# numericalEFT/FeynmanDiagram.jl

Hardware: AMD Instinct MI355X
Metric: graph-evaluations/sec (higher is better)
Workload: dtype f64

## Files before the change

### feynmandiagram.jl_amd/csrc/fdg_binned.hip

```cpp
#include <hip/hip_runtime.h>

#include <algorithm>
#include <cmath>
#include <mutex>
#include <type_traits>
#include <utility>
#include <vector>

#define FDG_RUNTIME_TU 1
#include "fdg_internal.h"
#include "fdg_matsubara.h"
#include "fdg_sincos.h"

using namespace fdg;

namespace {

constexpr uint32_t kBinWaves = 4;
constexpr size_t kBinLdsBudget = 64u << 10;
constexpr size_t kBinSlabBytes = 64ull << 20;
constexpr uint32_t kKeyInvalid = 0xFFFFFFC0u;

__device__ inline void bin_barrier() {
  __asm__ volatile("s_waitcnt lgkmcnt(0)\n\ts_barrier" ::: "memory");
}

__device__ inline uint32_t wave_sort_keys(uint32_t &key, uint32_t lane, uint64_t valid) {
  const uint32_t key0 = __shfl(key, 0);
  if (valid == ~0ull && __ballot((key >> 6) == (key0 >> 6)) == ~0ull) return lane;
#pragma unroll
  for (uint32_t kb = 2; kb <= 64; kb <<= 1)
#pragma unroll
    for (uint32_t jb = kb >> 1; jb > 0; jb >>= 1) {
      const uint32_t other = __shfl_xor(key, (int)jb);
      const bool keep_min = ((lane & kb) == 0) == ((lane & jb) == 0);
      key = keep_min ? min(key, other) : max(key, other);
    }
  return key & 63u;
}

__device__ inline void wave_runs(uint32_t key, uint32_t lane, uint32_t &j, bool &head, uint32_t &end) {
  j = key >> 6;
  const bool ok = key < kKeyInvalid;
  const uint32_t j_prev = __shfl_up(j, 1);
  const uint32_t j_next = __shfl_down(j, 1);
  head = ok && (lane == 0 || j_prev != j);
  const uint64_t tails = __ballot(!ok || lane == 63 || j_next != j);
  end = ok ? (uint32_t)__builtin_ctzll(tails & (~0ull << lane)) : lane;
}

struct SegTiles { long t0, t1, rounds; };
__device__ inline SegTiles seg_tiles_of(long n, uint32_t seg, long seg_tiles) {
  const long ntile = (n + 63) / 64, t0 = (long)seg * seg_tiles, t1 = min(t0 + seg_tiles, ntile);
  return {t0, t1, t1 > t0 ? (t1 - t0 + kBinWaves - 1) / kBinWaves : 0};
}

enum BinMode { kFirst = 0, kBoth = 1, kSplit = 2 };

constexpr uint32_t kGrpCols = FDG_WEIGHT_GROUP_MAX, kGrpEntry = 1u + kGrpCols + 16u;

template <int RS, int MODE, bool GRP = false>
__global__ void __launch_bounds__(256)
fdg_binned_partials(const double *__restrict__ root, long ld, long n, const int32_t *__restrict__ bins, int32_t bin_base, uint32_t n_bin,
                    const double *__restrict__ weight, uint32_t R, uint32_t n_slice, long seg_tiles, double *__restrict__ partial, int first,
                    const uint32_t *__restrict__ gtab, long wstride) {
  extern __shared__ double hist[];
  constexpr uint32_t NH = MODE == kBoth ? 2 : 1;
  const uint32_t lane = threadIdx.x & 63u, wave = threadIdx.x >> 6;
  const uint32_t n_grp = MODE == kSplit ? 2 * n_slice : n_slice;
  const uint32_t grp = blockIdx.x % n_grp, seg = blockIdx.x / n_grp;
  const uint32_t mom = MODE == kSplit ? grp / n_slice : 0, slice = grp % n_slice;
  const uint32_t k0 = slice * RS, kn = min((uint32_t)RS, R - k0);
  const size_t hist_cols = (size_t)n_bin * R;
  double *slab = partial + (size_t)seg * hist_cols * (MODE == kFirst ? 1 : 2) + (size_t)mom * hist_cols + k0;
  for (uint32_t i = threadIdx.x; i < NH * n_bin * RS; i += 256) {
    const uint32_t j = i / RS, kk = i % RS;
    hist[i] = (first || kk >= kn) ? 0.0 : slab[(size_t)j * R + kk];
  }
  __syncthreads();
  const SegTiles sg = seg_tiles_of(n, seg, seg_tiles);
  const long t0 = sg.t0, t1 = sg.t1, rounds = sg.rounds;

  constexpr int WC = !GRP ? 1 : RS < (int)kGrpCols ? RS : (int)kGrpCols;
  uint32_t n_wcol = 1, wcol[WC] = {}, widx[RS] = {};
  if constexpr (GRP) {
    const uint32_t *e = gtab + R + (size_t)slice * kGrpEntry;
    n_wcol = e[0];
#pragma unroll
    for (int c = 0; c < WC; ++c) wcol[c] = e[1 + c];
#pragma unroll
    for (int kk = 0; kk < RS; ++kk) widx[kk] = e[1 + kGrpCols + kk];
  }
  int32_t bin_n;
  double w_n[WC] = {}, r_n[RS];
  auto fetch = [&](long r) {
    const long b = min((t0 + r * (long)kBinWaves + wave) * 64 + lane, n - 1);
    bin_n = bins ? bins[b] : bin_base;
    if constexpr (GRP) {
#pragma unroll
      for (int c = 0; c < WC; ++c)
        if ((uint32_t)c < n_wcol) w_n[c] = weight[(size_t)wcol[c] * (size_t)wstride + (size_t)b];
    } else {
      w_n[0] = weight ? weight[b] : 1.0;
    }
#pragma unroll
    for (int kk = 0; kk < RS; ++kk) r_n[kk] = root[(size_t)min(k0 + kk, R - 1) * (size_t)ld + (size_t)b];
  };
  fetch(0);
  for (long r = 0; r < rounds; ++r) {
    const long t = t0 + r * (long)kBinWaves + wave, b = t * 64 + lane;
    const int64_t jb = (int64_t)bin_n - (int64_t)bin_base;
    const bool in = t < t1 && b < n && jb >= 0 && jb < (int64_t)n_bin;
    uint32_t key = in ? ((uint32_t)jb << 6) | lane : kKeyInvalid | lane;
    double v[RS];
#pragma unroll
    for (int kk = 0; kk < RS; ++kk) {
      double wk = w_n[0];
#pragma unroll
      for (int c = 1; c < WC; ++c) wk = widx[kk] == (uint32_t)c ? w_n[c] : wk;
      v[kk] = in ? wk * r_n[kk] : 0.0;
    }
    fetch(r + 1);

    const uint64_t valid = __ballot(key < kKeyInvalid);
    double s[RS] = {}, s2[RS] = {};
    bool head = false;
    uint32_t j = 0;
    if (valid) {
      const uint32_t src = wave_sort_keys(key, lane, valid);
      uint32_t end;
      wave_runs(key, lane, j, head, end);
#pragma unroll
      for (int kk = 0; kk < RS; ++kk) s[kk] = __shfl(v[kk], (int)src);
      if (MODE == kBoth) {
#pragma unroll
        for (int kk = 0; kk < RS; ++kk) s2[kk] = s[kk] * s[kk];
      } else if (MODE == kSplit && mom) {
#pragma unroll
        for (int kk = 0; kk < RS; ++kk) s[kk] = s[kk] * s[kk];
      }
      for (uint32_t d = 1; d < 64; d <<= 1) {
        const bool take = lane + d <= end;
        if (!__ballot(take)) break;
#pragma unroll
        for (int kk = 0; kk < RS; ++kk) {
          const double t = __shfl_down(s[kk], d);
          if (take) s[kk] = s[kk] + t;
        }
        if (MODE == kBoth) {
#pragma unroll
          for (int kk = 0; kk < RS; ++kk) {
            const double t = __shfl_down(s2[kk], d);
            if (take) s2[kk] = s2[kk] + t;
          }
        }
      }
    }
    for (uint32_t w = 0; w < kBinWaves; ++w) {
      if (wave == w && head) {
#pragma unroll
        for (int kk = 0; kk < RS; ++kk)
          if ((uint32_t)kk < kn) {
            hist[j * RS + kk] = hist[j * RS + kk] + s[kk];
            if (MODE == kBoth) hist[(n_bin + j) * RS + kk] = hist[(n_bin + j) * RS + kk] + s2[kk];
          }
      }
      bin_barrier();
    }
  }
  __syncthreads();
  for (uint32_t i = threadIdx.x; i < NH * n_bin * RS; i += 256) {
    const uint32_t jj = i / RS, kk = i % RS;
    if (kk < kn) slab[(size_t)jj * R + kk] = hist[i];
  }
}

__global__ void __launch_bounds__(256)
fdg_binned_reduce(const double *__restrict__ partial, uint32_t n_seg, long seg_stride, long ncol, uint32_t R, uint32_t C,
                  double *__restrict__ acc, double *__restrict__ acc2, const uint8_t *__restrict__ live) {
  __shared__ double sh[256];
  const uint32_t Q = 256u / C, q = threadIdx.x / C, cl = threadIdx.x % C;
  const long c = (long)blockIdx.x * C + cl;
  const double *part = partial + (size_t)blockIdx.y * (size_t)ncol;
  double *out = blockIdx.y ? acc2 : acc;
  double s = 0.0;
  if (c < ncol)
    for (uint32_t sg = q; sg < n_seg; sg += Q) s = s + part[(size_t)sg * (size_t)seg_stride + (size_t)c];
  sh[threadIdx.x] = s;
  __syncthreads();
  if (q == 0 && c < ncol) {
    double t = sh[cl];
    for (uint32_t qq = 1; qq < Q && qq < n_seg; ++qq) t = t + sh[qq * C + cl];
    if (!live || live[c % R]) out[c] = out[c] + t;
  }
}

constexpr uint32_t kObsGroup = 16;
constexpr uint32_t kObsNone = 0xFFFFFFFFu;
constexpr uint32_t kObsFirst = 0x80000000u;

__global__ void __launch_bounds__(256)
fdg_obs_partials(const double *__restrict__ root, long ld, long n, const int32_t *__restrict__ bins, int32_t bin_base, uint32_t n_bin,
                 const double *__restrict__ weight, long wstride, uint32_t n_wcol, uint32_t V, uint32_t CS, uint32_t n_slice, long seg_tiles,
                 double *__restrict__ partial, int first, const uint32_t *__restrict__ utab, const double *__restrict__ dtab) {
  extern __shared__ double hist[];
  const uint32_t lane = threadIdx.x & 63u, wave = threadIdx.x >> 6;
  const uint32_t slice = blockIdx.x % n_slice, seg = blockIdx.x / n_slice;
  const uint32_t c0 = slice * CS, cn = min(CS, V - c0);
  const uint32_t *hdr = utab + (size_t)slice * 4u;
  const uint32_t n_rec = hdr[1];
  const uint32_t *colA = utab + hdr[2], *colB = colA + CS, *rec = colB + CS, *tslot = rec + (size_t)n_rec * 4u;
  const double *tcoef = dtab + hdr[3];
  double *stash = hist + (size_t)n_bin * CS + threadIdx.x;
  double *slab = partial + (size_t)seg * n_bin * V + c0;
  for (uint32_t i = threadIdx.x; i < n_bin * CS; i += 256) {
    const uint32_t j = i / CS, cl = i % CS;
    hist[i] = (first || cl >= cn) ? 0.0 : slab[(size_t)j * V + cl];
  }
  __syncthreads();
  const SegTiles sg = seg_tiles_of(n, seg, seg_tiles);
  const long t0 = sg.t0, t1 = sg.t1, rounds = sg.rounds;
  int32_t bin_n;
  auto fetch = [&](long r) {
    const long b = min((t0 + r * (long)kBinWaves + wave) * 64 + lane, n - 1);
    bin_n = bins ? bins[b] : bin_base;
  };
  fetch(0);
  for (long r = 0; r < rounds; ++r) {
    const long t = t0 + r * (long)kBinWaves + wave, b = t * 64 + lane;
    const int64_t jb = (int64_t)bin_n - (int64_t)bin_base;
    const bool in = t < t1 && b < n && jb >= 0 && jb < (int64_t)n_bin;
    uint32_t key = in ? ((uint32_t)jb << 6) | lane : kKeyInvalid | lane;
    fetch(r + 1);
    const uint64_t valid = __ballot(key < kKeyInvalid);
    bool head = false, ok = false;
    uint32_t j = 0, end = lane;
    if (valid) {
      const uint32_t src = wave_sort_keys(key, lane, valid);
      wave_runs(key, lane, j, head, end);
      ok = key < kKeyInvalid;
      const size_t bs = (size_t)min(t * 64 + (long)src, n - 1);
      double wv[kGrpCols] = {};
#pragma unroll
      for (uint32_t c = 0; c < kGrpCols; ++c)
        if (c < n_wcol) wv[c] = weight[(size_t)c * (size_t)wstride + bs];
      for (uint32_t i0 = 0; i0 < n_rec; i0 += 4) {
        double rv[4];
#pragma unroll
        for (uint32_t u = 0; u < 4; ++u) rv[u] = root[(size_t)rec[(size_t)min(i0 + u, n_rec - 1u) * 4u] * (size_t)ld + bs];
#pragma unroll
        for (uint32_t u = 0; u < 4; ++u) {
          if (i0 + u >= n_rec) break;
          const uint32_t *e = rec + (size_t)(i0 + u) * 4u;
          const uint32_t wc = e[1];
          double wk = wv[0];
#pragma unroll
          for (uint32_t c = 1; c < kGrpCols; ++c) wk = wc == c ? wv[c] : wk;
          const double tk = n_wcol ? wk * rv[u] : rv[u];
          for (uint32_t ti = e[2]; ti < e[3]; ++ti) {
            const uint32_t sl = tslot[ti];
            double *o = stash + (size_t)(sl & ~kObsFirst) * 256u;
            const double p = tcoef[ti] * tk;
            *o = (sl & kObsFirst) ? p : *o + p;
          }
        }
      }
    }
    for (uint32_t g0 = 0; g0 < cn; g0 += kObsGroup) {
      double s[kObsGroup];
      if (valid) {
#pragma unroll
        for (uint32_t i = 0; i < kObsGroup; ++i) {
          const uint32_t cl = min(g0 + i, cn - 1u), a = colA[cl], c = colB[cl];
          double v = 0.0;
          if (a != kObsNone) {
            v = stash[(size_t)a * 256u];
            if (c != kObsNone) v = v * stash[(size_t)c * 256u];
          }
          s[i] = ok ? v : 0.0;
        }
        for (uint32_t d = 1; d < 64; d <<= 1) {
          const bool take = lane + d <= end;
          if (!__ballot(take)) break;
#pragma unroll
          for (uint32_t i = 0; i < kObsGroup; ++i) {
            const double up = __shfl_down(s[i], d);
            if (take) s[i] = s[i] + up;
          }
        }
      }
      for (uint32_t w = 0; w < kBinWaves; ++w) {
        if (wave == w && head) {
#pragma unroll
          for (uint32_t i = 0; i < kObsGroup; ++i)
            if (g0 + i < cn) hist[(size_t)j * CS + g0 + i] = hist[(size_t)j * CS + g0 + i] + s[i];
        }
        bin_barrier();
      }
    }
  }
  __syncthreads();
  for (uint32_t i = threadIdx.x; i < n_bin * CS; i += 256) {
    const uint32_t jj = i / CS, cl = i % CS;
    if (cl < cn) slab[(size_t)jj * V + cl] = hist[i];
  }
}

__global__ void __launch_bounds__(256)
fdg_obs_reduce(const double *__restrict__ partial, uint32_t n_seg, long ncol, uint32_t n_obs, uint32_t V, uint32_t C, uint32_t rowlive,
               double *__restrict__ obs, double *__restrict__ cov) {
  __shared__ double sh[256];
  const uint32_t Q = 256u / C, q = threadIdx.x / C, cl = threadIdx.x % C;
  const long c = (long)blockIdx.x * C + cl;
  double s = 0.0;
  if (c < ncol)
    for (uint32_t sg = q; sg < n_seg; sg += Q) s = s + partial[(size_t)sg * (size_t)ncol + (size_t)c];
  sh[threadIdx.x] = s;
  __syncthreads();
  if (q == 0 && c < ncol) {
    double t = sh[cl];
    for (uint32_t qq = 1; qq < Q && qq < n_seg; ++qq) t = t + sh[qq * C + cl];
    const size_t jb = (size_t)(c / V);
    const uint32_t v = (uint32_t)(c % V);
    if (v < n_obs) {
      if ((rowlive >> v) & 1u) obs[jb * n_obs + v] = obs[jb * n_obs + v] + t;
    } else {
      uint32_t a = 0, p = v - n_obs;
      while (p >= n_obs - a) { p -= n_obs - a; ++a; }
      const uint32_t cc = a + p;
      if (((rowlive >> a) & 1u) && ((rowlive >> cc) & 1u)) {
        double *m = cov + jb * n_obs * n_obs;
        const double up = m[a * n_obs + cc] + t;
        m[a * n_obs + cc] = up;
        if (cc != a) m[cc * n_obs + a] = m[cc * n_obs + a] + t;
      }
    }
  }
}

constexpr uint32_t kFobsRec = 6;
constexpr uint32_t kFobsSame = 0x80000000u;
constexpr uint32_t kFobsIm = 0x40000000u;

__global__ void __launch_bounds__(256)
fdg_fobs_partials(const double *__restrict__ root, long ld, long n, const int32_t *__restrict__ bins, int32_t bin_base, uint32_t n_bin,
                  const double *__restrict__ weight, long wstride, uint32_t n_wcol, const double *__restrict__ T, long ts, long tc,
                  double beta, uint32_t n_freq, uint32_t FS, uint32_t n_fslice, uint32_t V, uint32_t CS, uint32_t n_cslice, long seg_tiles,
                  double *__restrict__ partial, int first, const uint32_t *__restrict__ utab, const double *__restrict__ dtab) {
  extern __shared__ double hist[];
  const uint32_t lane = threadIdx.x & 63u, wave = threadIdx.x >> 6;
  const uint32_t n_grp = n_fslice * n_cslice, grp = blockIdx.x % n_grp, seg = blockIdx.x / n_grp;
// ... 126 lines not shown
                double *__restrict__ fobs, double *__restrict__ fcov) {
  __shared__ double sh[256];
  const uint32_t Q = 256u / C, q = threadIdx.x / C, cl = threadIdx.x % C;
  const long c = (long)blockIdx.x * C + cl;
  double s = 0.0;
  if (c < ncol)
    for (uint32_t sg = q; sg < n_seg; sg += Q) s = s + partial[(size_t)sg * (size_t)ncol + (size_t)c];
  sh[threadIdx.x] = s;
  __syncthreads();
  if (q == 0 && c < ncol) {
    double t = sh[cl];
    for (uint32_t qq = 1; qq < Q && qq < n_seg; ++qq) t = t + sh[qq * C + cl];
    const size_t row = (size_t)(c / V);
    const uint32_t v = (uint32_t)(c % V);
    if (v < n_comp) {
      if ((live >> v) & 1u) fobs[row * n_comp + v] = fobs[row * n_comp + v] + t;
    } else {
      uint32_t a = 0, p = v - n_comp;
      while (p >= n_comp - a) { p -= n_comp - a; ++a; }
      const uint32_t cc = a + p;
      if (((live >> a) & 1u) && ((live >> cc) & 1u)) {
        double *m = fcov + row * n_comp * n_comp;
        m[a * n_comp + cc] = m[a * n_comp + cc] + t;
        if (cc != a) m[cc * n_comp + a] = m[cc * n_comp + a] + t;
      }
    }
  }
}

__device__ __forceinline__ uint32_t vegas_cell(uint64_t sample, uint32_t d, uint64_t seed, uint32_t G, double &y) {
  const double u = fdg_philox_u53(sample, d, seed);
  y = u * (double)G;
  return min((uint32_t)(int)y, G - 1u);
}

struct VegasStrat { uint32_t n[FDG_VEGAS_DIM_MAX], div[FDG_VEGAS_DIM_MAX], H; };

__device__ __forceinline__ uint32_t vegas_cell_strat(uint64_t sample, uint32_t d, uint64_t seed, uint32_t G, uint32_t s, uint32_t ns, double &y) {
  const double u = fdg_philox_u53(sample, d, seed);
  const double v = ((double)s + u) / (double)ns;
  y = v * (double)G;
  return min((uint32_t)(int)y, G - 1u);
}

struct VegasCols { uint32_t c[FDG_VEGAS_DIM_MAX]; };

struct VegasNoFold { __device__ void operator()(uint32_t, double) const {} };
struct VegasPlainCell {
  __device__ __forceinline__ uint32_t operator()(uint64_t sample, uint32_t d, uint64_t seed, uint32_t G, double &y) const {
    return vegas_cell(sample, d, seed, G, y);
  }
};
struct VegasStratCell {
  const VegasStrat *sv;
  uint32_t rem;
  __device__ __forceinline__ uint32_t operator()(uint64_t sample, uint32_t d, uint64_t seed, uint32_t G, double &y) {
    const uint32_t ns = sv->n[d], sd = rem % ns;
    rem /= ns;
    return vegas_cell_strat(sample, d, seed, G, sd, ns, y);
  }
};
template <bool kPolar = false, class Fold = VegasNoFold, class Cell = VegasPlainCell>
__device__ __forceinline__ double vegas_draw(const double *__restrict__ grid, uint32_t D, uint32_t G, const VegasCols &col, uint64_t seed,
                                             uint64_t off, double *__restrict__ x, long xs, long xc, int32_t *__restrict__ cell, long n, long b,
                                             uint64_t grouped = 0, double *stash = nullptr, Fold fold = Fold(), Cell pick = Cell()) {
  double jb = 0.0;
  uint32_t slot = 0;
  for (uint32_t d = 0; d < D; ++d) {
    double y;
    const uint32_t c = pick(off + (uint64_t)b, d, seed, G, y);
    const double *e = grid + (size_t)d * (G + 1u) + c;
    const double lo = e[0], wd = e[1] - lo, fr = y - (double)c;
    const double v = lo + fr * wd;
    if (kPolar && ((grouped >> d) & 1u)) stash[(slot++) * 256u + threadIdx.x] = v;
    else x[b * xs + (long)col.c[d] * xc] = v;
    const double f = (double)G * wd;
    jb = d ? jb * f : f;
    fold(d, f);
    if (cell) cell[(size_t)d * (size_t)n + (size_t)b] = (int32_t)c;
  }
  return jb;
}

__global__ void __launch_bounds__(256)
fdg_vegas_sample(const double *__restrict__ grid, uint32_t D, uint32_t G, VegasCols col, uint64_t seed, uint64_t off, double *__restrict__ x,
                 long xs, long xc, double *__restrict__ jac, int32_t *__restrict__ cell, long n) {
  for (long b = blockIdx.x * 256L + threadIdx.x; b < n; b += (long)gridDim.x * 256L) {
    const double jb = vegas_draw(grid, D, G, col, seed, off, x, xs, xc, cell, n, b);
    jac[b] = jb;
  }
}

__global__ void __launch_bounds__(256)
fdg_vegas_sample_strat(const double *__restrict__ grid, uint32_t D, uint32_t G, VegasCols col, VegasStrat sv, const int64_t *__restrict__ start,
                       uint64_t seed, uint64_t off, double *__restrict__ x, long xs, long xc, double *__restrict__ jac,
                       int32_t *__restrict__ cube, int32_t *__restrict__ cell, long n) {
  const uint32_t H = sv.H;
  const int64_t n_total = start[H];
  for (long b = blockIdx.x * 256L + threadIdx.x; b < n; b += (long)gridDim.x * 256L) {
    const int64_t i = (int64_t)(off + (uint64_t)b);
    uint32_t lo = 0, hi = H - 1u;
    while (lo < hi) {
      const uint32_t mid = (lo + hi + 1u) >> 1;
      if (start[mid] <= i) lo = mid; else hi = mid - 1u;
    }
    const int64_t n_h = start[lo + 1u] - start[lo];
    cube[b] = (int32_t)lo;
    uint32_t rem = lo;
    double jb = 0.0;
    for (uint32_t d = 0; d < D; ++d) {
      const uint32_t ns = sv.n[d], sd = rem % ns;
      rem /= ns;
      double y;
      const uint32_t c = vegas_cell_strat(off + (uint64_t)b, d, seed, G, sd, ns, y);
      const double *e = grid + (size_t)d * (G + 1u) + c;
      const double el = e[0], wd = e[1] - el, fr = y - (double)c;
      x[b * xs + (long)col.c[d] * xc] = el + fr * wd;
      const double f = (double)G * wd;
      jb = d ? jb * f : f;
      if (cell) cell[(size_t)d * (size_t)n + (size_t)b] = (int32_t)c;
    }
    const double fac = (double)n_total / ((double)H * (double)n_h);
    jac[b] = jb * fac;
  }
}

struct VegasExtCols { uint32_t c[FDG_VEGAS_EXT_MAX]; };

__device__ __forceinline__ double vegas_pick_discrete(const double *__restrict__ cdf, uint32_t n_bin, int32_t bin_base,
                                                      const double *__restrict__ ext, uint32_t n_ext, const VegasExtCols &ecol, uint64_t seed,
                                                      uint64_t off, uint32_t D, double *__restrict__ x, long xs, long xc,
                                                      int32_t *__restrict__ bin, long b) {
  const double u = fdg_philox_u53(off + (uint64_t)b, D, seed);
  uint32_t lo = 0, hi = n_bin - 1u;
  while (lo < hi) {
    const uint32_t mid = (lo + hi) >> 1;
    if (cdf[mid + 1u] <= u) lo = mid + 1u; else hi = mid;
  }
  const double p = cdf[lo + 1u] - cdf[lo];
  bin[b] = (int32_t)lo + bin_base;
  for (uint32_t e = 0; e < n_ext; ++e) x[b * xs + (long)ecol.c[e] * xc] = ext[(size_t)lo * n_ext + e];
  return p;
}

__device__ __forceinline__ void vegas_draw_discrete(const double *__restrict__ cdf, uint32_t n_bin, int32_t bin_base,
                                                    const double *__restrict__ ext, uint32_t n_ext, const VegasExtCols &ecol, uint64_t seed,
                                                    uint64_t off, uint32_t D, double *__restrict__ x, long xs, long xc,
                                                    double *__restrict__ jac, int32_t *__restrict__ bin, long b, double jb) {
  const double p = vegas_pick_discrete(cdf, n_bin, bin_base, ext, n_ext, ecol, seed, off, D, x, xs, xc, bin, b);
  jac[b] = jb / p;
}

__global__ void __launch_bounds__(256)
fdg_vegas_sample_discrete(const double *__restrict__ grid, uint32_t D, uint32_t G, VegasCols col, const double *__restrict__ cdf,
                          uint32_t n_bin, int32_t bin_base, const double *__restrict__ ext, uint32_t n_ext, VegasExtCols ecol, uint64_t seed,
                          uint64_t off, double *__restrict__ x, long xs, long xc, double *__restrict__ jac, int32_t *__restrict__ bin,
                          int32_t *__restrict__ cell, long n) {
  for (long b = blockIdx.x * 256L + threadIdx.x; b < n; b += (long)gridDim.x * 256L) {
    const double jb = vegas_draw(grid, D, G, col, seed, off, x, xs, xc, cell, n, b);
    vegas_draw_discrete(cdf, n_bin, bin_base, ext, n_ext, ecol, seed, off, D, x, xs, xc, jac, bin, b, jb);
  }
}

struct VegasPolar {
  uint64_t grouped;
  uint32_t n;
  uint32_t var[FDG_VEGAS_POLAR_MAX], dim[FDG_VEGAS_POLAR_MAX];
  uint32_t col[FDG_VEGAS_POLAR_MAX][3];
};

struct VegasGroupMasks {
  uint64_t m[FDG_WEIGHT_GROUP_MAX];
  uint32_t n;
};

struct VegasNoStrat {};
struct VegasStratArgs {
  VegasStrat sv;
  const int64_t *start;
  int32_t *cube;
};
template <bool GRP, bool STRAT = false>
__global__ void __launch_bounds__(256)
fdg_vegas_sample_polar(const double *__restrict__ grid, uint32_t D, uint32_t G, VegasCols col, VegasPolar pol, const double *__restrict__ cdf,
                       uint32_t n_bin, int32_t bin_base, const double *__restrict__ ext, uint32_t n_ext, VegasExtCols ecol, uint64_t seed,
                       uint64_t off, double *__restrict__ x, long xs, long xc, double *__restrict__ jac, int32_t *__restrict__ bin,
                       int32_t *__restrict__ cell, long n, VegasGroupMasks gm, long jstride,
                       std::conditional_t<STRAT, VegasStratArgs, VegasNoStrat> sa) {
  extern __shared__ double polar_stash[];
  constexpr int NG = GRP ? FDG_WEIGHT_GROUP_MAX : 1;
  for (long b = blockIdx.x * 256L + threadIdx.x; b < n; b += (long)gridDim.x * 256L) {
    [[maybe_unused]] double fac = 1.0;
    [[maybe_unused]] uint32_t hcube = 0;
    if constexpr (STRAT) {
      const uint32_t H = sa.sv.H;
      const int64_t i = (int64_t)(off + (uint64_t)b);
      uint32_t lo = 0, hi = H - 1u;
      while (lo < hi) {
        const uint32_t mid = (lo + hi + 1u) >> 1;
        if (sa.start[mid] <= i) lo = mid; else hi = mid - 1u;
      }
      const int64_t n_h = sa.start[lo + 1u] - sa.start[lo];
      sa.cube[b] = (int32_t)lo;
      hcube = lo;
      fac = (double)sa.start[H] / ((double)H * (double)n_h);
    }
    double jg[NG];
#pragma unroll
    for (int g = 0; g < NG; ++g) jg[g] = 1.0;
    auto fold = [&](uint32_t d, double f) {
      if constexpr (GRP) {
#pragma unroll
        for (int g = 0; g < NG; ++g)
          if ((uint32_t)g < gm.n && ((gm.m[g] >> d) & 1u)) jg[g] = jg[g] * f;
      }
    };
    double jb;
    if constexpr (STRAT) jb = vegas_draw<true>(grid, D, G, col, seed, off, x, xs, xc, cell, n, b, pol.grouped, polar_stash, fold, VegasStratCell{&sa.sv, hcube});
    else jb = vegas_draw<true>(grid, D, G, col, seed, off, x, xs, xc, cell, n, b, pol.grouped, polar_stash, fold);
    for (uint32_t g = 0; g < pol.n; ++g) {
      const uint32_t var = pol.var[g];
      const double *v = polar_stash + (size_t)__popcll(pol.grouped & ((1ull << var) - 1ull)) * 256u + threadIdx.x;
      double *xb = x + b * xs;
      const double k = v[0];
      double sp, cp, st = 0.0;
      if (pol.dim[g] == 3) {
        double ct;
        fdg_sincos_impl(v[256], st, ct);
        fdg_sincos_impl(v[512], sp, cp);
        const double ks = k * st;
        xb[(long)pol.col[g][0] * xc] = ks * cp;
        xb[(long)pol.col[g][1] * xc] = ks * sp;
        xb[(long)pol.col[g][2] * xc] = k * ct;
        jb = jb * k;
        jb = jb * k;
        jb = jb * st;
      } else {
        fdg_sincos_impl(v[256], sp, cp);
        xb[(long)pol.col[g][0] * xc] = k * cp;
        xb[(long)pol.col[g][1] * xc] = k * sp;
        jb = jb * k;
      }
      if constexpr (GRP) {
#pragma unroll
        for (int h = 0; h < NG; ++h)
          if ((uint32_t)h < gm.n && ((gm.m[h] >> var) & 1u)) {
            jg[h] = jg[h] * k;
            if (pol.dim[g] == 3) {
              jg[h] = jg[h] * k;
              jg[h] = jg[h] * st;
            }
          }
      }
    }
    if constexpr (STRAT) {
      if constexpr (GRP) {
#pragma unroll
        for (int g = 0; g < NG; ++g)
          if ((uint32_t)g < gm.n) jac[(size_t)g * (size_t)jstride + (size_t)b] = jg[g] * fac;
      } else {
        jac[b] = jb * fac;
      }
    } else if constexpr (GRP) {
      const double p = cdf ? vegas_pick_discrete(cdf, n_bin, bin_base, ext, n_ext, ecol, seed, off, D, x, xs, xc, bin, b) : 1.0;
#pragma unroll
      for (int g = 0; g < NG; ++g)
        if ((uint32_t)g < gm.n) jac[(size_t)g * (size_t)jstride + (size_t)b] = cdf ? jg[g] / p : jg[g];
    } else {
      if (!cdf) { jac[b] = jb; continue; }
      vegas_draw_discrete(cdf, n_bin, bin_base, ext, n_ext, ecol, seed, off, D, x, xs, xc, jac, bin, b, jb);
    }
  }
}

__device__ __forceinline__ double vegas_term(const double *__restrict__ root, long ld, size_t bb, const double *__restrict__ weight,
                                             const uint32_t *__restrict__ kidx, const double *__restrict__ coef, uint32_t n_live) {
  double sum = 0.0;
  for (uint32_t i = 0; i < n_live; ++i) {
    const double rk = root[(size_t)kidx[i] * (size_t)ld + bb];
    const double term = coef ? coef[i] * rk : rk;
    sum = i ? sum + term : term;
  }
  return weight ? weight[bb] * sum : sum;
}

__device__ __forceinline__ double vegas_group_term(const double *__restrict__ root, long ld, size_t bb, const double *__restrict__ weight,
                                                   long wstride, const uint32_t *__restrict__ kidx, const double *__restrict__ coef,
                                                   const uint32_t *__restrict__ gstart, uint32_t g) {
  const uint32_t i0 = gstart[g], i1 = gstart[g + 1u];
  return vegas_term(root, ld, bb, weight + (size_t)g * (size_t)wstride, kidx + i0, coef ? coef + i0 : nullptr, i1 - i0);
}

struct VegasVarGroups { uint8_t g[FDG_VEGAS_DIM_MAX]; };

template <int BINNED, bool GRP = false, bool STRAT = false>
__global__ void __launch_bounds__(256)
fdg_vegas_partials(const double *__restrict__ root, long ld, long n, const double *__restrict__ weight, const uint32_t *__restrict__ kidx,
                   const double *__restrict__ coef, uint32_t n_live, uint64_t seed, uint64_t off, uint32_t D, uint32_t G, uint32_t DS,
                   uint32_t n_slice, long seg_tiles, double *__restrict__ partial, int first, const int32_t *__restrict__ bins,
                   int32_t bin_base, uint32_t n_bin, const uint32_t *__restrict__ gstart, uint32_t NG, long wstride, VegasVarGroups vgm,
                   const int32_t *__restrict__ cube, VegasStrat sv) {
  extern __shared__ double hist[];
  const uint32_t vtile = GRP ? NG * 64u : 64u;
  const uint32_t lane = threadIdx.x & 63u, wave = threadIdx.x >> 6;
  const uint32_t slice = blockIdx.x % n_slice, seg = blockIdx.x / n_slice;
  const uint32_t d0 = slice * DS, dn = min(DS, D - d0);
  double *vbuf = hist + (size_t)DS * G;
  double *slab = partial + ((size_t)seg * D + d0) * G;
  for (uint32_t i = threadIdx.x; i < dn * G; i += 256) hist[i] = first ? 0.0 : slab[i];
  __syncthreads();
  const SegTiles sg = seg_tiles_of(n, seg, seg_tiles);
  const long t0 = sg.t0, t1 = sg.t1, rounds = sg.rounds;
  for (long r = 0; r < rounds; ++r) {
    {
      const long t = t0 + r * (long)kBinWaves + wave, b = t * 64 + lane;
      bool in = t < t1 && b < n;
      const size_t bb = (size_t)min(b, n - 1);
      if (BINNED) {
        const int64_t jb = (int64_t)bins[bb] - (int64_t)bin_base;
        in = in && jb >= 0 && jb < (int64_t)n_bin;
      }
      const double out = (BINNED && t < t1 && b < n) ? -1.0 : 0.0;
      double *vb = vbuf + ((r & 1) * kBinWaves + wave) * vtile + lane;
      if constexpr (GRP) {
        for (uint32_t g = 0; g < NG; ++g) {
          const double tw = vegas_group_term(root, ld, bb, weight, wstride, kidx, coef, gstart, g);
          vb[g * 64u] = in ? tw * tw : out;
        }
      } else {
        const double tw = vegas_term(root, ld, bb, weight, kidx, coef, n_live);
        vb[0] = in ? tw * tw : out;
      }
    }
    __syncthreads();
    for (uint32_t tt = 0; tt < kBinWaves; ++tt) {
      const long t = t0 + r * (long)kBinWaves + tt, b = t * 64 + lane;
      if (t >= t1) break;
      const double *vb = vbuf + ((r & 1) * kBinWaves + tt) * vtile + lane;
      double v = GRP ? 0.0 : vb[0];
      uint32_t hc = 0;
      if constexpr (STRAT) hc = (uint32_t)cube[(size_t)min(b, n - 1)];
      for (uint32_t dd = wave; dd < dn; dd += kBinWaves) {
        if constexpr (GRP) {
          const uint32_t owners = vgm.g[d0 + dd];
          if (!owners) continue;
          bool any = false;
          for (uint32_t g = 0; g < NG; ++g)
            if ((owners >> g) & 1u) {
              const double q = vb[g * 64u];
              v = any ? v + q : q;
              any = true;
            }
        }
        double y;
        uint32_t c;
        if constexpr (STRAT) c = vegas_cell_strat(off + (uint64_t)b, d0 + dd, seed, G, hc / sv.div[d0 + dd] % sv.n[d0 + dd], sv.n[d0 + dd], y);
        else c = vegas_cell(off + (uint64_t)b, d0 + dd, seed, G, y);
        uint32_t key = (b < n && !(STRAT && hc >= sv.H) && !(BINNED && v < 0.0)) ? (c << 6) | lane : kKeyInvalid | lane;
        const uint64_t valid = __ballot(key < kKeyInvalid);
        if (!valid) continue;
        const uint32_t src = wave_sort_keys(key, lane, valid);
        uint32_t j, end;
        bool head;
        wave_runs(key, lane, j, head, end);
        double s = __shfl(v, (int)src);
        for (uint32_t dist = 1; dist < 64; dist <<= 1) {
          const bool take = lane + dist <= end;
          if (!__ballot(take)) break;
          const double up = __shfl_down(s, dist);
          if (take) s = s + up;
        }
        if (head) hist[dd * G + j] = hist[dd * G + j] + s;
      }
    }
  }
  __syncthreads();
  for (uint32_t i = threadIdx.x; i < dn * G; i += 256) slab[i] = hist[i];
}

template <bool GRP = false>
__global__ void __launch_bounds__(256)
fdg_vegas_bin_partials(const double *__restrict__ root, long ld, long n, const int32_t *__restrict__ bins, int32_t bin_base, uint32_t n_bin,
                       const double *__restrict__ weight, const uint32_t *__restrict__ kidx, const double *__restrict__ coef, uint32_t n_live,
                       long seg_tiles, double *__restrict__ partial, int first, const uint32_t *__restrict__ gstart, uint32_t NG,
                       long wstride) {
  extern __shared__ double hist[];
  const uint32_t lane = threadIdx.x & 63u, wave = threadIdx.x >> 6;
  const uint32_t seg = blockIdx.x;
  double *slab = partial + (size_t)seg * n_bin;
  for (uint32_t i = threadIdx.x; i < n_bin; i += 256) hist[i] = first ? 0.0 : slab[i];
  __syncthreads();
  const SegTiles sg = seg_tiles_of(n, seg, seg_tiles);
  const long t0 = sg.t0, t1 = sg.t1, rounds = sg.rounds;
  int32_t bin_n;
  double t_n = 0.0;
  auto fetch = [&](long r) {
    const size_t bb = (size_t)min((t0 + r * (long)kBinWaves + wave) * 64 + lane, n - 1);
    bin_n = bins[bb];
    if constexpr (GRP) {
      bool any = false;
      for (uint32_t g = 0; g < NG; ++g) {
        if (gstart[g] == gstart[g + 1u]) continue;
        const double tw = vegas_group_term(root, ld, bb, weight, wstride, kidx, coef, gstart, g), q = tw * tw;
        t_n = any ? t_n + q : q;
        any = true;
      }
    } else {
      t_n = vegas_term(root, ld, bb, weight, kidx, coef, n_live);
    }
  };
  fetch(0);
  for (long r = 0; r < rounds; ++r) {
    const long t = t0 + r * (long)kBinWaves + wave, b = t * 64 + lane;
    const int64_t jb = (int64_t)bin_n - (int64_t)bin_base;
    const bool in = t < t1 && b < n && jb >= 0 && jb < (int64_t)n_bin;
    uint32_t key = in ? ((uint32_t)jb << 6) | lane : kKeyInvalid | lane;
    const double v = in ? (GRP ? t_n : t_n * t_n) : 0.0;
    fetch(r + 1);
    const uint64_t valid = __ballot(key < kKeyInvalid);
    double s = 0.0;
    bool head = false;
    uint32_t j = 0;
    if (valid) {
      const uint32_t src = wave_sort_keys(key, lane, valid);
      uint32_t end;
      wave_runs(key, lane, j, head, end);
      s = __shfl(v, (int)src);
      for (uint32_t dist = 1; dist < 64; dist <<= 1) {
        const bool take = lane + dist <= end;
        if (!__ballot(take)) break;
        const double up = __shfl_down(s, dist);
        if (take) s = s + up;
      }
    }
    for (uint32_t w = 0; w < kBinWaves; ++w) {
      if (wave == w && head) hist[j] = hist[j] + s;
      bin_barrier();
    }
  }
  __syncthreads();
  for (uint32_t i = threadIdx.x; i < n_bin; i += 256) slab[i] = hist[i];
}

template <int KW, bool HSPLIT, bool GRP = false>
__global__ void __launch_bounds__(256)
fdg_matsubara_partials(const double *__restrict__ root, long ld, long n, const int32_t *__restrict__ bins, int32_t bin_base, uint32_t n_bin,
                       const double *__restrict__ weight, const double *__restrict__ T, long ts, long tc, const double *__restrict__ tab,
                       double beta, uint32_t n_freq, uint32_t R, uint32_t RS, uint32_t FS, uint32_t n_fslice, long seg_tiles,
                       double *__restrict__ partial, int first, const uint32_t *__restrict__ rgrp, long wstride) {
  extern __shared__ double hist[];
  constexpr uint32_t NH = HSPLIT ? 1 : 4;
  const uint32_t lane = threadIdx.x & 63u, wave = threadIdx.x >> 6, nw = blockDim.x >> 6;
  const uint32_t n_rslice = (R + RS - 1) / RS, n_grp = n_rslice * n_fslice * (HSPLIT ? 4u : 1u);
  const uint32_t grp = blockIdx.x % n_grp, seg = blockIdx.x / n_grp;
  const uint32_t h0 = HSPLIT ? grp / (n_rslice * n_fslice) : 0u;
  const uint32_t fslice = (grp / n_rslice) % n_fslice, rslice = grp % n_rslice;
  const uint32_t k0 = rslice * RS, kn = min(RS, R - k0), fb = fslice * FS, fn = min(FS, n_freq - fb);
  const size_t ncol = (size_t)n_bin * n_freq * R;
  double *slab = partial + ((size_t)seg * 4u + h0) * ncol;
  const uint32_t per = n_bin * FS * RS;
  auto slab_at = [&](uint32_t i, bool &live) {
    const uint32_t kk = i % RS, fl = (i / RS) % FS, j = (i / (RS * FS)) % n_bin, hh = i / per;
    live = kk < kn && fl < fn;
    return (size_t)hh * ncol + ((size_t)j * n_freq + fb + fl) * R + k0 + kk;
  };
  for (uint32_t i = threadIdx.x; i < NH * per; i += blockDim.x) {
    bool live;
    const size_t at = slab_at(i, live);
    hist[i] = (first || !live) ? 0.0 : slab[at];
  }
  __syncthreads();
  const SegTiles sg = seg_tiles_of(n, seg, seg_tiles);
  const uint32_t kk0 = RS >= nw ? wave : wave % RS, f0 = RS >= nw ? 0u : wave / RS, fstep = RS >= nw ? 1u : nw / RS;
  const int32_t *tio = (const int32_t *)(tab + FDG_MATSUBARA_FREQ_MAX);
  long off_in[KW], off_out[KW];
  size_t col[KW], wcol[KW] = {};
  int wfrom[KW] = {};
#pragma unroll
  for (int m = 0; m < KW; ++m) {
    const uint32_t k = min(k0 + kk0 + nw * (uint32_t)m, R - 1u);
    col[m] = (size_t)k * (size_t)ld;
    if constexpr (GRP) {
      wcol[m] = (size_t)rgrp[k] * (size_t)wstride;
      wfrom[m] = m;
#pragma unroll
      for (int e = m - 1; e >= 0; --e)
        if (wcol[e] == wcol[m]) wfrom[m] = e;
    }
    off_in[m] = (long)tio[k] * tc;
    off_out[m] = (long)tio[R + k] * tc;
  }
  if (kk0 < kn && f0 < fn) {
    int32_t bin_n;
    double w_n[GRP ? KW : 1] = {}, r_n[KW], ti_n[KW], to_n[KW];
    auto fetch = [&](long t) {
      const size_t bb = (size_t)min(t * 64 + (long)lane, n - 1);
      bin_n = bins ? bins[bb] : bin_base;
      if constexpr (!GRP) w_n[0] = weight ? weight[bb] : 1.0;
#pragma unroll
      for (int m = 0; m < KW; ++m) {
        if constexpr (GRP)
          if (wfrom[m] == m) w_n[m] = weight[wcol[m] + bb];
        r_n[m] = root[col[m] + bb];
        ti_n[m] = T[(long)bb * ts + off_in[m]];
        to_n[m] = T[(long)bb * ts + off_out[m]];
      }
    };
    fetch(sg.t0);
    for (long t = sg.t0; t < sg.t1; ++t) {
      const long b = t * 64 + lane;
      const int64_t jb = (int64_t)bin_n - (int64_t)bin_base;
      const bool in = b < n && jb >= 0 && jb < (int64_t)n_bin;
      uint32_t key = in ? ((uint32_t)jb << 6) | lane : kKeyInvalid | lane;
      double tv[KW], xv[KW];
#pragma unroll
      for (int m = 0; m < KW; ++m) {
        const double tau = to_n[m] - ti_n[m];
        double wk = w_n[0];
        if constexpr (GRP) {
#pragma unroll
          for (int e = 1; e <= m; ++e) wk = wfrom[m] == e ? w_n[e] : wk;
        }
        tv[m] = in ? wk * r_n[m] : 0.0;
        xv[m] = in ? tau / beta : 0.0;
      }
      fetch(min(t + 1, sg.t1 - 1));
      const uint64_t valid = __ballot(key < kKeyInvalid);
      if (!valid) continue;
      const uint32_t src = wave_sort_keys(key, lane, valid);
      uint32_t j, end;
      bool head;
      wave_runs(key, lane, j, head, end);
#pragma unroll
      for (int m = 0; m < KW; ++m) {
        const uint32_t kk = kk0 + nw * (uint32_t)m;
        if (kk >= kn) break;
        const double ts_ = __shfl(tv[m], (int)src), xs = __shfl(xv[m], (int)src);
        for (uint32_t fl = f0; fl < fn; fl += fstep) {
          double s, c;
          matsubara_phase_of(xs, tab[fb + fl], s, c);
          const double tre = ts_ * c, tim = ts_ * s;
          double v[NH];
          if constexpr (HSPLIT) {
            v[0] = h0 == 0 ? tre : h0 == 1 ? tim : h0 == 2 ? tre * tre : tim * tim;
          } else {
            v[0] = tre;
            v[1] = tim;
            v[2] = tre * tre;
            v[3] = tim * tim;
          }
          for (uint32_t d = 1; d < 64; d <<= 1) {
            const bool take = lane + d <= end;
            if (!__ballot(take)) break;
#pragma unroll
            for (uint32_t hh = 0; hh < NH; ++hh) {
              const double up = __shfl_down(v[hh], d);
              if (take) v[hh] = v[hh] + up;
            }
          }
          if (head) {
            double *hw = hist + ((size_t)j * FS + fl) * RS + kk;
#pragma unroll
            for (uint32_t hh = 0; hh < NH; ++hh) hw[(size_t)hh * per] = hw[(size_t)hh * per] + v[hh];
          }
        }
      }
    }
  }
  __syncthreads();
  for (uint32_t i = threadIdx.x; i < NH * per; i += blockDim.x) {
    bool live;
    const size_t at = slab_at(i, live);
    if (live) slab[at] = hist[i];
  }
}

constexpr uint32_t kStratCols = 8, kStratVals = 2 * kStratCols;

__device__ __forceinline__ uint32_t strat_wmask(uint32_t k0, uint32_t R, uint32_t E, const uint8_t *__restrict__ live, uint32_t emask) {
  uint32_t m = 0;
  for (uint32_t j = 0; j < kStratVals; ++j) {
    const uint32_t kk = k0 + (j & (kStratCols - 1u));
    const bool on = kk < R ? (!live || live[kk]) : (kk - R < E && ((emask >> (kk - R)) & 1u) != 0);
    m |= on ? 1u << j : 0u;
  }
  return m;
}

__device__ __forceinline__ void strat_wave_reduce(int32_t key, bool ok, uint32_t lane, double (&s)[kStratVals], uint32_t k0, uint32_t C1,
                                                  uint32_t wmask, double *__restrict__ sum, double *__restrict__ sum2, bool final,
                                                  int32_t *__restrict__ rkey, double *__restrict__ rval, long rstride, long slot) {
  const bool wkey = blockIdx.y == 0;
  const uint64_t valid = __ballot(ok);
  if (!valid) {
    if (!final && wkey && lane < 2) rkey[slot + lane] = -1;
    return;
  }
  const uint64_t upto = valid & (lane == 63 ? ~0ull : ((2ull << lane) - 1ull));
  const int src = upto ? 63 - __builtin_clzll(upto) : __builtin_ctzll(valid);
  const int32_t kf = __shfl(key, src);
  const int32_t k_prev = __shfl_up(kf, 1), k_next = __shfl_down(kf, 1);
  const bool head = lane == 0 || k_prev != kf;
  const uint64_t tails = __ballot(lane == 63 || k_next != kf);
  const uint32_t end = (uint32_t)__builtin_ctzll(tails & (~0ull << lane));
  for (uint32_t d = 1; d < 64; d <<= 1) {
    const bool take = lane + d <= end;
    if (!__ballot(take)) break;
#pragma unroll
    for (uint32_t j = 0; j < kStratVals; ++j) {
      const double up = __shfl_down(s[j], d);
      if (take) s[j] = s[j] + up;
    }
  }
  if (!head) return;
  const bool at0 = lane == 0, at63 = end == 63;
  if (final || (!at0 && !at63)) {
#pragma unroll
    for (uint32_t j = 0; j < kStratVals; ++j)
      if ((wmask >> j) & 1u) {
        double *o = (j < kStratCols ? sum : sum2) + (size_t)kf * C1 + k0 + (j & (kStratCols - 1u));
        *o = *o + s[j];
      }
    return;
  }
  const long at = slot + (at0 ? 0 : 1);
  if (wkey) rkey[at] = kf;
  if (wkey && at0 && at63) rkey[at + 1] = kf;
#pragma unroll
  for (uint32_t j = 0; j < kStratVals; ++j) {
    const uint32_t kk = k0 + (j & (kStratCols - 1u));
    if (kk >= C1) continue;
    double *o = rval + (size_t)((j < kStratCols ? 0u : C1) + kk) * (size_t)rstride + (size_t)at;
    o[0] = s[j];
    if (at0 && at63) o[1] = 0.0;
  }
}

template <bool GRP = false>
__global__ void __launch_bounds__(256)
fdg_strat_partials(const double *__restrict__ root, long ld, long n, const int32_t *__restrict__ cube, uint32_t H,
                   const double *__restrict__ weight, const uint32_t *__restrict__ kidx, const double *__restrict__ coef, uint32_t n_live,
                   uint32_t R, const uint8_t *__restrict__ live, double *__restrict__ sum, double *__restrict__ sum2,
                   int32_t *__restrict__ rkey, double *__restrict__ rval, long rstride, long slot_base,
                   const uint32_t *__restrict__ rgrp, const uint32_t *__restrict__ gstart, uint32_t NG, long wstride, uint32_t emask) {
  const uint32_t lane = threadIdx.x & 63u, wave = threadIdx.x >> 6;
  const long t = (long)blockIdx.x * kBinWaves + wave;
  if (t >= (n + 63) / 64) return;
  const uint32_t E = GRP ? NG : 1u;
  const uint32_t k0 = blockIdx.y * kStratCols, C1 = R + E;
  const long b = t * 64 + lane;
  const size_t bb = (size_t)min(b, n - 1);
  const int32_t h = cube[bb];
  const bool ok = b < n && (uint32_t)h < H;
  double w = 1.0;
  if constexpr (!GRP) w = weight ? weight[bb] : 1.0;
  double s[kStratVals];
#pragma unroll
  for (uint32_t i = 0; i < kStratCols; ++i) {
    const uint32_t kk = k0 + i;
    double tk = 0.0;
    if constexpr (GRP) {
      if (kk < R) tk = weight[(size_t)rgrp[kk] * (size_t)wstride + bb] * __builtin_nontemporal_load(root + (size_t)kk * (size_t)ld + bb);
      else if (kk < C1) tk = vegas_group_term(root, ld, bb, weight, wstride, kidx, coef, gstart, kk - R);
    } else {
      if (kk < R) tk = w * __builtin_nontemporal_load(root + (size_t)kk * (size_t)ld + bb);
      else if (kk == R) tk = vegas_term(root, ld, bb, weight, kidx, coef, n_live);
    }
    s[i] = ok ? tk : 0.0;
    s[kStratCols + i] = ok ? tk * tk : 0.0;
  }
// ... 1522 lines not shown
```

Before: 9.332 billion.

## Replace wave bitonic sort with ballot-based peer matching for small VEGAS histogram runs

In the VEGAS partials kernel, each lane now finds the lanes sharing its grid cell by taking one ballot per bit of the cell index. If no cell has more than eight contributors, the lowest matching lane gathers the peers' values through LDS reads or shuffles, sums them with a fixed tree, and adds the result to the histogram, so the full 64-lane bitonic sort and segmented scan are skipped. The sort path remains as a fallback for larger runs. The change also makes the wave index uniform with readfirstlane and moves the tile loop counters to 32-bit. The cost is log2(G) ballots per dimension and extra branching, which may exceed the sort's cost when G is large or runs are long.

```diff
diff --git a/feynmandiagram.jl_amd/csrc/fdg_binned.hip b/feynmandiagram.jl_amd/csrc/fdg_binned.hip
--- a/feynmandiagram.jl_amd/csrc/fdg_binned.hip
+++ b/feynmandiagram.jl_amd/csrc/fdg_binned.hip
@@ -47,6 +47,32 @@
   head = ok && (lane == 0 || j_prev != j);
   const uint64_t tails = __ballot(!ok || lane == 63 || j_next != j);
   end = ok ? (uint32_t)__builtin_ctzll(tails & (~0ull << lane)) : lane;
+}
+
+constexpr uint32_t kMatchRun = 8;
+__device__ __forceinline__ uint64_t wave_peers(uint32_t c, uint32_t nbit, uint64_t valid) {
+  uint64_t m = valid;
+  for (uint32_t k = 0; k < nbit; ++k) {
+    const bool bit = (c >> k) & 1u;
+    const uint64_t bk = __ballot(bit);
+    m &= bit ? bk : ~bk;
+  }
+  return m;
+}
+
+__device__ __forceinline__ double run_sum4(double a, double b, double c, double d, uint32_t m) {
+  const double ab = a + b, cd = c + d;
+  const double x = m >= 2u ? ab : a;
+  const double y = x + (m == 3u ? c : cd);
+  return m >= 3u ? y : x;
+}
+
+__device__ __forceinline__ double run_sum(const double (&e)[kMatchRun], uint32_t n) {
+  static_assert(kMatchRun == 8, "run_sum spells the tree out for runs of up to 8");
+  const double lo = run_sum4(e[0], e[1], e[2], e[3], min(n, 4u));
+  const double hi = run_sum4(e[4], e[5], e[6], e[7], n - 4u);
+  const double both = lo + hi;
+  return n > 4u ? both : lo;
 }
 
 struct SegTiles { long t0, t1, rounds; };
@@ -779,7 +805,7 @@
                    const int32_t *__restrict__ cube, VegasStrat sv) {
   extern __shared__ double hist[];
   const uint32_t vtile = GRP ? NG * 64u : 64u;
-  const uint32_t lane = threadIdx.x & 63u, wave = threadIdx.x >> 6;
+  const uint32_t lane = threadIdx.x & 63u, wave = (uint32_t)__builtin_amdgcn_readfirstlane((int)(threadIdx.x >> 6));
   const uint32_t slice = blockIdx.x % n_slice, seg = blockIdx.x / n_slice;
   const uint32_t d0 = slice * DS, dn = min(DS, D - d0);
   double *vbuf = hist + (size_t)DS * G;
@@ -787,10 +813,12 @@
   for (uint32_t i = threadIdx.x; i < dn * G; i += 256) hist[i] = first ? 0.0 : slab[i];
   __syncthreads();
   const SegTiles sg = seg_tiles_of(n, seg, seg_tiles);
-  const long t0 = sg.t0, t1 = sg.t1, rounds = sg.rounds;
-  for (long r = 0; r < rounds; ++r) {
+  const uint32_t t0 = (uint32_t)sg.t0, t1 = (uint32_t)sg.t1, rounds = (uint32_t)sg.rounds;
+  const uint32_t nbit = G > 1u ? 32u - (uint32_t)__builtin_clz(G - 1u) : 0u;
+  for (uint32_t r = 0; r < rounds; ++r) {
     {
-      const long t = t0 + r * (long)kBinWaves + wave, b = t * 64 + lane;
+      const uint32_t t = t0 + r * kBinWaves + wave;
+      const long b = (long)t * 64 + lane;
       bool in = t < t1 && b < n;
       const size_t bb = (size_t)min(b, n - 1);
       if (BINNED) {
@@ -811,12 +839,15 @@
     }
     __syncthreads();
     for (uint32_t tt = 0; tt < kBinWaves; ++tt) {
-      const long t = t0 + r * (long)kBinWaves + tt, b = t * 64 + lane;
+      const uint32_t t = t0 + r * kBinWaves + tt;
+      const long b = (long)t * 64 + lane;
       if (t >= t1) break;
-      const double *vb = vbuf + ((r & 1) * kBinWaves + tt) * vtile + lane;
+      const double *vrow = vbuf + ((r & 1u) * kBinWaves + tt) * vtile, *vb = vrow + lane;
       double v = GRP ? 0.0 : vb[0];
       uint32_t hc = 0;
       if constexpr (STRAT) hc = (uint32_t)cube[(size_t)min(b, n - 1)];
+      bool live = b < n;
+      if constexpr (STRAT) live = live && hc < sv.H;
       for (uint32_t dd = wave; dd < dn; dd += kBinWaves) {
         if constexpr (GRP) {
           const uint32_t owners = vgm.g[d0 + dd];
@@ -833,16 +864,37 @@
         uint32_t c;
         if constexpr (STRAT) c = vegas_cell_strat(off + (uint64_t)b, d0 + dd, seed, G, hc / sv.div[d0 + dd] % sv.n[d0 + dd], sv.n[d0 + dd], y);
         else c = vegas_cell(off + (uint64_t)b, d0 + dd, seed, G, y);
-        uint32_t key = (b < n && !(STRAT && hc >= sv.H) && !(BINNED && v < 0.0)) ? (c << 6) | lane : kKeyInvalid | lane;
-        const uint64_t valid = __ballot(key < kKeyInvalid);
+        const bool ok = live && !(BINNED && v < 0.0);
+        const uint64_t valid = __ballot(ok);
         if (!valid) continue;
-        const uint32_t src = wave_sort_keys(key, lane, valid);
+        const uint64_t peers = wave_peers(c, nbit, valid);
+        const uint32_t cnt = (uint32_t)__popcll(peers);
+        if (!__ballot(ok && cnt > kMatchRun)) {
+          const bool head1 = ok && __builtin_amdgcn_mbcnt_hi((uint32_t)(peers >> 32), __builtin_amdgcn_mbcnt_lo((uint32_t)peers, 0u)) == 0u;
+          uint64_t rest = head1 ? peers & (peers - 1ull) : 0ull;
+          double e[kMatchRun] = {v};
+#pragma unroll
+          for (uint32_t i = 1; i < kMatchRun; ++i) {
+            if (!__ballot(rest != 0ull)) break;
+            const uint32_t at = rest ? (uint32_t)__builtin_ctzll(rest) : lane;
+            rest &= rest - 1ull;
+            if constexpr (GRP) e[i] = __shfl(v, (int)at);
+            else e[i] = vrow[at];
+          }
+          const double s1 = run_sum(e, cnt);
+          if (head1) hist[dd * G + c] = hist[dd * G + c] + s1;
+          continue;
+        }
+        uint32_t ln = lane;
+        __asm__ volatile("" : "+v"(ln));
+        uint32_t key = ok ? (c << 6) | ln : kKeyInvalid | ln;
+        const uint32_t src = wave_sort_keys(key, ln, valid);
         uint32_t j, end;
         bool head;
-        wave_runs(key, lane, j, head, end);
+        wave_runs(key, ln, j, head, end);
         double s = __shfl(v, (int)src);
         for (uint32_t dist = 1; dist < 64; dist <<= 1) {
-          const bool take = lane + dist <= end;
+          const bool take = ln + dist <= end;
           if (!__ballot(take)) break;
           const double up = __shfl_down(s, dist);
           if (take) s = s + up;
```

After: 9.269 billion. No clear change (-0.7%).
